# wg-perception/PartsBasedDetector

Measured on AMD Instinct MI355X. Metric: detect() frames/sec, 640x480, 26-part person model, higher is better.
Workload: dtype f32

## Files before the change

### partsbaseddetector_amd/csrc/k_conv_split32.hpp

```cpp
typedef __bf16 bf16x8 __attribute__((ext_vector_type(8)));
typedef _Float16 f16x8 __attribute__((ext_vector_type(8)));
typedef unsigned u32x4 __attribute__((ext_vector_type(4)));
typedef float f32x4 __attribute__((ext_vector_type(4)));
typedef float f32x16 __attribute__((ext_vector_type(16)));

template <int NT, int NW, int PIN, int NS = 3, bool MIX = false>
__global__ __launch_bounds__(64 * NW) __attribute__((amdgpu_waves_per_eu(1, PIN ? 1 : 2))) void k_conv_split32(const ConvTile* __restrict__ tiles, const LevelDev* __restrict__ levels,
                                                             const uint16_t* __restrict__ feat, const uint16_t* __restrict__ filt,
                                                             float* __restrict__ resp, int nf, int ntl_bank, int ntile0, int ngroups,
                                                             int ntiles_total, int kh, int kw, const float* __restrict__ oscale) {
  extern __shared__ __attribute__((aligned(16))) char smem[];
  using opnd = std::conditional_t<NS == 3, bf16x8, f16x8>;
  constexpr int ROWS = 4 * NW, NHALVES = 16 / ROWS, NTHR = 64 * NW, PPC = 4 * NS;
  const int TW = 16 + kw - 1, TH = ROWS + kh - 1, NC = TW * TH, PLANE = NC * 64;
  const int R = NHALVES * ngroups;
  const int lin = blockIdx.x;
  const int grp = lin / (8 * R), rem = lin - grp * (8 * R);
  const int tile_i = grp * 8 + (rem & 7), role = rem >> 3;
  if (tile_i >= ntiles_total) return;
  const int half = role & (NHALVES - 1), ngroup = role / NHALVES;
  const ConvTile t = tiles[tile_i];
  const LevelDev lv = levels[t.level];
  const int H = lv.ch, W = lv.cw;
  const int ty0 = t.y0 + ROWS * half, tx0 = t.x0;
  if (ty0 >= H) return;
  const int tid = threadIdx.x, lane = tid & 63, wave = __builtin_amdgcn_readfirstlane(tid >> 6);
  const uint16_t* F = feat + lv.cell_off * (NS * PBD_FLEN);
  {
    const int NPC = NC * PPC, oy = ty0 - kh / 2, ox = tx0 - kw / 2;
    constexpr unsigned ONE = NS == 3 ? 0x3F800000u : 0x6C000000u;
    auto cell_of = [](int i) { return NS == 3 ? (int)(((unsigned)i * 43691u) >> 19) : i >> 3; };
    const unsigned magic_tw = 0xFFFFFFFFu / (unsigned)TW + 1u;
    constexpr int BATCH = 12;
    for (int i0 = 0; i0 < NPC; i0 += NTHR * BATCH) {
      u32x4 v[BATCH];
#pragma unroll
      for (int j = 0; j < BATCH; ++j) {
        const int i = min(i0 + j * NTHR + tid, NPC - 1);
        const int cell = cell_of(i), piece = i - cell * PPC;
        const int cy = (int)__umulhi((unsigned)cell, magic_tw), cx = cell - cy * TW;
        const int y = min(max(oy + cy, 0), H - 1), x = min(max(ox + cx, 0), W - 1);
        v[j] = *(const u32x4*)(F + ((size_t)(y * W + x) * (NS * PBD_FLEN) + piece * 8));
      }
#pragma unroll
      for (int j = 0; j < BATCH; ++j) {
        const int i = i0 + j * NTHR + tid;
        if (i < NPC) {
          const int cell = cell_of(i), piece = i - cell * PPC;
          const int cy = (int)__umulhi((unsigned)cell, magic_tw), cx = cell - cy * TW;
          const int y = oy + cy, x = ox + cx;
          const bool inside = y >= 0 && y < H && x >= 0 && x < W;
          const u32x4 border = u32x4{0u, 0u, 0u, piece == 3 ? ONE : 0u};
          const int q = piece & 3;
          *(u32x4*)(smem + (piece >> 2) * PLANE + cell * 64 + ((q ^ ((cell >> 2) & 3)) << 4)) = inside ? v[j] : border;
        }
      }
    }
  }
  __syncthreads();
  const int c = lane & 31, kg = lane >> 5;
  const int mid = ((c & 15) >= 4 && (c & 15) < 12) ? 1 : 0;
  const int pos = (c & 15) + 16 * (mid ^ (c >> 4));
  const int vw = min(16, W - tx0), vh = min(ROWS, H - ty0), ncell = vw * vh;
  const int nmt = (ncell + 31) >> 5;
  const int mvalid = __builtin_amdgcn_readfirstlane(max(0, min(2, (nmt - wave + NW - 1) / NW)));
  const unsigned vw_magic = 65535u / (unsigned)vw + 1u;
  int cl0[2], cofs[2];
  bool cval[2];
#pragma unroll
  for (int m = 0; m < 2; ++m) {
    const int idx = 32 * (wave + NW * m) + pos;
    cval[m] = idx < ncell;
    const int ic = min(idx, ncell - 1);
    const int cy = (int)(((unsigned)ic * vw_magic) >> 16), cx = ic - cy * vw;
    cl0[m] = cy * TW + cx;
    cofs[m] = (ty0 + cy) * W + tx0 + cx;
  }
  const int ntb = ntile0 + ngroup * NT;
  f32x16 acc[NT][2];
#pragma unroll
  for (int nt = 0; nt < NT; ++nt)
#pragma unroll
    for (int m = 0; m < 2; ++m)
#pragma unroll
      for (int r = 0; r < 16; ++r) acc[nt][m][r] = 0.f;
  const uint16_t* bl = filt + (size_t)ntb * 512 + lane * 8;
  const size_t bs_split = (size_t)ntl_bank * 512, bs_kstep = NS * bs_split;
  const int nkstep = 2 * kh * kw;
#ifdef PBD_BANK_PRIO
  __builtin_amdgcn_s_setprio(PBD_BANK_PRIO);
#endif

  auto k_loop = [&](auto mv_tag) __attribute__((always_inline)) {
    constexpr int MV = decltype(mv_tag)::value;
    auto load_b = [&](opnd (&b)[NT][NS], int kstep) __attribute__((always_inline)) {
      const uint16_t* p = bl + (size_t)min(kstep, nkstep - 1) * bs_kstep;
#pragma unroll
      for (int s = 0; s < NS; ++s)
#pragma unroll
        for (int nt = 0; nt < NT; ++nt) b[nt][s] = *(const opnd*)(p + s * bs_split + nt * 512);
    };
    auto load_a = [&](opnd (&a)[2][NS], int tapofs, int ks) __attribute__((always_inline)) {
#pragma unroll
      for (int m = 0; m < MV; ++m) {
        const int cl = cl0[m] + tapofs;
        const char* p = smem + cl * 64 + (((2 * ks + kg) ^ ((cl >> 2) & 3)) << 4);
#pragma unroll
        for (int s = 0; s < NS; ++s) a[m][s] = *(const opnd*)(p + s * PLANE);
      }
    };
    auto mma = [&](const opnd (&a)[2][NS], const opnd (&b)[NT][NS]) __attribute__((always_inline)) {
      auto sweep = [&](int sa, int sb) __attribute__((always_inline)) {
#pragma unroll
        for (int nt = 0; nt < NT; ++nt)
#pragma unroll
          for (int m = 0; m < MV; ++m) {
            if constexpr (NS == 3) acc[nt][m] = __builtin_amdgcn_mfma_f32_32x32x16_bf16(b[nt][sb], a[m][sa], acc[nt][m], 0, 0, 0);
            else acc[nt][m] = __builtin_amdgcn_mfma_f32_32x32x16_f16(b[nt][sb], a[m][sa], acc[nt][m], 0, 0, 0);
          }
      };
      if constexpr (NS == 3) { sweep(1, 1); sweep(0, 2); sweep(2, 0); }
      sweep(0, 1); sweep(1, 0); sweep(0, 0);
    };
    int ti = 0, tj = 0;
    const int ntap = kh * kw;
    opnd a0[2][NS], a1[2][NS], b0[NT][NS], b1[NT][NS];
    load_b(b0, 0);
    load_a(a0, 0, 0);
#pragma unroll 1
    for (int tap = 0; tap < ntap; ++tap) {
      const int tapofs = ti * TW + tj;
      auto deal = [&]() {
        if constexpr (PIN == 2) {
#pragma unroll
          for (int i = 0; i < NS * NT; ++i) { __builtin_amdgcn_sched_group_barrier(0x8, NS == 3 ? (MV == 2 ? 3 : 1) : MV, 0); __builtin_amdgcn_sched_group_barrier(0x20, 1, 0); }
#pragma unroll
          for (int i = 0; i < NS * MV; ++i) { __builtin_amdgcn_sched_group_barrier(0x8, 2, 0); __builtin_amdgcn_sched_group_barrier(0x100, 1, 0); }
        }
      };
      if (PIN) __builtin_amdgcn_sched_barrier(0);
      load_b(b1, 2 * tap + 1);
      load_a(a1, tapofs, 1);
      if (PIN == 1) __builtin_amdgcn_sched_barrier(0);
      mma(a0, b0);
      deal();
      if (PIN) __builtin_amdgcn_sched_barrier(0);
      if (++tj == kw) { tj = 0; ++ti; }
      const int nextofs = tap + 1 < ntap ? ti * TW + tj : tapofs;
      load_b(b0, 2 * tap + 2);
      load_a(a0, nextofs, 0);
      if (PIN == 1) __builtin_amdgcn_sched_barrier(0);
      mma(a1, b1);
      deal();
      if (PIN) __builtin_amdgcn_sched_barrier(0);
    }
  };
  if (mvalid == 2) k_loop(std::integral_constant<int, 2>());
  else if (mvalid == 1) k_loop(std::integral_constant<int, 1>());
  if (mvalid == 0) return;

  float* Rl = resp + lv.cell_off * nf;
  const size_t HW = (size_t)H * W;
  int nfw = nf;
  if constexpr (MIX) { Rl += (size_t)(t.pad & 0xFFFF) * HW; nfw = t.pad >> 16; }
#pragma unroll
  for (int m = 0; m < 2; ++m) {
    if (m < mvalid && cval[m]) {
#pragma unroll
      for (int nt = 0; nt < NT; ++nt) {
        float* pl = Rl + (size_t)(32 * (ntb + nt) + 4 * kg) * HW + cofs[m];
#pragma unroll
        for (int r = 0; r < 16; ++r) {
          const int fo = (r & 3) + 8 * (r >> 2);
          if (32 * (ntb + nt) + 4 * kg + fo < nfw) pl[(size_t)fo * HW] = NS == 3 ? acc[nt][m][r] : acc[nt][m][r] * oscale[32 * (ntb + nt) + 4 * kg + fo];
        }
      }
    }
  }
}

template <int NT, int NW, int PIN, int NS = 3, bool MIX = false>
static void launch_conv_split_t(const ConvTile* tiles, int ntiles, const LevelDev* levels, const uint16_t* feat_split, const uint16_t* wS,
                                float* resp, int nf, int ntl_bank, int ntile0, int ngroups, int kh, int kw, hipStream_t s, const float* oscale = nullptr,
                                int nf_stride = 0) {
  constexpr int ROWS = 4 * NW, NHALVES = 16 / ROWS;
  const size_t lds = (size_t)(16 + kw - 1) * (ROWS + kh - 1) * 64 * NS;
  static LdsOptIn optin;
  optin.ensure((const void*)k_conv_split32<NT, NW, PIN, NS, MIX>, lds);
  const int grid = (ntiles + 7) / 8 * 8 * NHALVES * ngroups;
  hipLaunchKernelGGL((k_conv_split32<NT, NW, PIN, NS, MIX>), dim3(grid), dim3(64 * NW), lds, s, tiles, levels, feat_split, wS, resp, MIX ? nf_stride : nf,
                     ntl_bank, ntile0, ngroups, ntiles, kh, kw, oscale);
}
template <int NW, int PIN, int NS, bool MIX = false>
static void launch_conv_split_groups(const ConvTile* tiles, int ntiles, const LevelDev* levels, const uint16_t* feat_split, const uint16_t* wS,
                                     float* resp, int nf, int kh, int kw, const float* oscale, hipStream_t s, int nf_stride = 0, int G = 5) {
  const int ntl = conv_split_ntiles(nf), full = ntl / G, rest = ntl - G * full;
  auto go = [&](int nt, int ntile0, int ngroups) {
    switch (nt) {
      case 1: launch_conv_split_t<1, NW, PIN, NS, MIX>(tiles, ntiles, levels, feat_split, wS, resp, nf, ntl, ntile0, ngroups, kh, kw, s, oscale, nf_stride); break;
      case 2: launch_conv_split_t<2, NW, PIN, NS, MIX>(tiles, ntiles, levels, feat_split, wS, resp, nf, ntl, ntile0, ngroups, kh, kw, s, oscale, nf_stride); break;
      case 3: launch_conv_split_t<3, NW, PIN, NS, MIX>(tiles, ntiles, levels, feat_split, wS, resp, nf, ntl, ntile0, ngroups, kh, kw, s, oscale, nf_stride); break;
      case 4: launch_conv_split_t<4, NW, PIN, NS, MIX>(tiles, ntiles, levels, feat_split, wS, resp, nf, ntl, ntile0, ngroups, kh, kw, s, oscale, nf_stride); break;
      case 5: launch_conv_split_t<5, NW, PIN, NS, MIX>(tiles, ntiles, levels, feat_split, wS, resp, nf, ntl, ntile0, ngroups, kh, kw, s, oscale, nf_stride); break;
      default: break;
    }
  };
  if (full) go(G, 0, full);
  if (rest) go(rest, G * full, 1);
}
```

### partsbaseddetector_amd/csrc/k_conv_split_variants.hip

```cpp
#include <algorithm>
#include <type_traits>
#include "pbd_internal.hpp"

int conv_split_ntiles(int nf);

namespace conv_variants {
#include "k_conv_split32.hpp"

template <int NT>
__device__ __forceinline__ void conv_split32p_body(char* smem, const ConvTile* __restrict__ tiles, const LevelDev* __restrict__ levels,
                                                   const uint16_t* __restrict__ feat, const uint16_t* __restrict__ filt,
                                                   float* __restrict__ resp, int nf, int ntl_bank, int ntile0, int ngroups,
                                                   int ntiles_total) {
  constexpr int NW = 4, KW = 5, TW = 20, NC = 400, HPLANE = NC * 32, HBUF = 3 * HPLANE, NTAP = 25, NHP = NC * 6;
  const int tid = threadIdx.x, lane = tid & 63, wave = __builtin_amdgcn_readfirstlane(tid >> 6);
  const int xcd = blockIdx.x & 7, j0 = blockIdx.x >> 3, nwx = gridDim.x >> 3;
  const int ntx = ntiles_total > xcd ? (ntiles_total - xcd + 7) >> 3 : 0;
  const int nunits = ntx * ngroups;
  if (j0 >= nunits) return;
  const int c = lane & 31, kg = lane >> 5;
  const int mid = ((c & 15) >= 4 && (c & 15) < 12) ? 1 : 0;
  const int pos = (c & 15) + 16 * (mid ^ (c >> 4));
  const size_t bs_split = (size_t)ntl_bank * 512, bs_kstep = 3 * bs_split;

  struct Unit { int y0, x0, W, H, ng; size_t cell_off; };
  auto unit_of = [&](int v) {
    const int ti = xcd + 8 * (v / ngroups);
    const ConvTile t = tiles[ti];
    const LevelDev lv = levels[t.level];
    return Unit{t.y0, t.x0, lv.cw, lv.ch, v - (v / ngroups) * ngroups, (size_t)lv.cell_off};
  };
  auto piece_src = [&](const Unit& U, int half, int jj) {
    const int i = min(jj * 256 + tid, NHP - 1);
    const int cell = (int)(((unsigned)i * 43691u) >> 18), p6 = i - cell * 6;
    const int cy = (int)(((unsigned)cell * 52429u) >> 20), cx = cell - cy * TW;
    const int y = min(max(U.y0 - 2 + cy, 0), U.H - 1), x = min(max(U.x0 - 2 + cx, 0), U.W - 1);
    const int gp = (p6 >> 1) * 4 + 2 * half + (p6 & 1);
    return (const u32x4*)(feat + (U.cell_off + (size_t)(y * U.W + x)) * (3 * PBD_FLEN) + gp * 8);
  };
  auto piece_put = [&](const Unit& U, int half, int jj, char* buf, u32x4 v) {
    const int i = min(jj * 256 + tid, NHP - 1);
    const int cell = (int)(((unsigned)i * 43691u) >> 18), p6 = i - cell * 6;
    const int cy = (int)(((unsigned)cell * 52429u) >> 20), cx = cell - cy * TW;
    const int y = U.y0 - 2 + cy, x = U.x0 - 2 + cx;
    const unsigned m = 0u - (unsigned)((int)(y >= 0) & (int)(y < U.H) & (int)(x >= 0) & (int)(x < U.W));
    const unsigned b3 = (half == 1 && p6 == 1) ? 0x3F800000u : 0u;
    const u32x4 w = u32x4{v[0] & m, v[1] & m, v[2] & m, (v[3] & m) | (b3 & ~m)};
    *(u32x4*)(buf + (p6 >> 1) * HPLANE + cell * 32 + (((p6 & 1) ^ ((cell >> 3) & 1)) << 4)) = w;
  };
  constexpr int NPT = (NHP + 255) / 256;
  static_assert(2 * NPT <= NTAP - 1, "a half tile is staged under the 25 k-steps of the previous half");

  int v = j0;
  Unit U = unit_of(v);
  {
    u32x4 r[NPT];
#pragma unroll
    for (int jj = 0; jj < NPT; ++jj) r[jj] = *piece_src(U, 0, jj);
#pragma unroll
    for (int jj = 0; jj < NPT; ++jj) piece_put(U, 0, jj, smem, r[jj]);
  }
  const uint16_t* bl = filt + (size_t)(ntile0 + U.ng * NT) * 512 + lane * 8;
  bf16x8 a0[2][3], a1[2][3], b0[NT][3], b1[NT][3];
  auto load_b = [&](bf16x8 (&b)[NT][3], const uint16_t* p) {
#pragma unroll
    for (int s = 0; s < 3; ++s)
#pragma unroll
      for (int nt = 0; nt < NT; ++nt) b[nt][s] = *(const bf16x8*)(p + s * bs_split + nt * 512);
  };
  load_b(b0, bl);
  f32x16 acc[NT][2];

  while (true) {
    const int vn = v + nwx;
    const bool has_next = vn < nunits;
    const Unit Un = unit_of(has_next ? vn : v);
    const uint16_t* bln = filt + (size_t)(ntile0 + Un.ng * NT) * 512 + lane * 8;
    const int vw = min(16, U.W - U.x0), vh = min(16, U.H - U.y0), ncell = vw * vh;
    const int nmt = (ncell + 31) >> 5;
    const int mvalid = __builtin_amdgcn_readfirstlane(max(0, min(2, (nmt - wave + NW - 1) / NW)));
    const unsigned vw_magic = 65535u / (unsigned)vw + 1u;
    int cl0[2], cofs[2];
    bool cval[2];
#pragma unroll
    for (int m = 0; m < 2; ++m) {
      const int idx = 32 * (wave + NW * m) + pos;
      cval[m] = idx < ncell;
      const int ic = min(idx, ncell - 1);
      const int cy = (int)(((unsigned)ic * vw_magic) >> 16), cx = ic - cy * vw;
      cl0[m] = cy * TW + cx;
      cofs[m] = (U.y0 + cy) * U.W + U.x0 + cx;
    }
#pragma unroll
    for (int nt = 0; nt < NT; ++nt)
#pragma unroll
      for (int m = 0; m < 2; ++m)
#pragma unroll
        for (int r = 0; r < 16; ++r) acc[nt][m][r] = 0.f;

    auto run_half = [&](auto mv_tag, int half, const char* bufc, char* bufn, const Unit& Us, int hs, const uint16_t* bnext,
                        bf16x8 (&ac)[2][3], bf16x8 (&bc)[NT][3], bf16x8 (&an)[2][3], bf16x8 (&bn)[NT][3]) __attribute__((always_inline)) {
      constexpr int MV = decltype(mv_tag)::value;
      auto load_a = [&](bf16x8 (&a)[2][3], int tapofs) {
#pragma unroll
        for (int m = 0; m < (MV ? MV : 1); ++m) {
          if (MV == 0) break;
          const int cl = cl0[m] + tapofs;
          const char* p = bufc + cl * 32 + ((kg ^ ((cl >> 3) & 1)) << 4);
#pragma unroll
          for (int s = 0; s < 3; ++s) a[m][s] = *(const bf16x8*)(p + s * HPLANE);
        }
      };
      auto mma = [&](const bf16x8 (&a)[2][3], const bf16x8 (&b)[NT][3]) {
        auto sweep = [&](int sa, int sb) {
#pragma unroll
          for (int nt = 0; nt < NT; ++nt)
#pragma unroll
            for (int m = 0; m < MV; ++m) acc[nt][m] = __builtin_amdgcn_mfma_f32_32x32x16_bf16(b[nt][sb], a[m][sa], acc[nt][m], 0, 0, 0);
        };
        sweep(1, 1); sweep(0, 2); sweep(2, 0); sweep(0, 1); sweep(1, 0); sweep(0, 0);
      };
      auto deal = [&](int extra_vmem, int extra_dsw) {
        if constexpr (MV > 0) {
#pragma unroll
          for (int i = 0; i < 3 * NT; ++i) { __builtin_amdgcn_sched_group_barrier(0x8, MV == 2 ? 3 : 1, 0); __builtin_amdgcn_sched_group_barrier(0x20, 1, 0); }
          if (extra_vmem) { __builtin_amdgcn_sched_group_barrier(0x8, 1, 0); __builtin_amdgcn_sched_group_barrier(0x20, 1, 0); }
          if (extra_dsw) { __builtin_amdgcn_sched_group_barrier(0x8, 1, 0); __builtin_amdgcn_sched_group_barrier(0x200, 1, 0); }
#pragma unroll
          for (int i = 0; i < 3 * MV; ++i) { __builtin_amdgcn_sched_group_barrier(0x8, MV == 2 ? 2 : 1, 0); __builtin_amdgcn_sched_group_barrier(0x100, 1, 0); }
        }
      };
      const uint16_t* bh = bl + (size_t)half * bs_kstep;
      __syncthreads();
      load_a(ac, 0);
      u32x4 pv = u32x4{0u, 0u, 0u, 0u};
      int ti = 0, tj = 0;
#pragma unroll 1
      for (int tp = 0; tp < NTAP / 2; ++tp) {
        __builtin_amdgcn_sched_barrier(0);
        pv = *piece_src(Us, hs, min(tp, NPT - 1));
        if (MV) load_b(bn, bh + (size_t)(2 * (2 * tp + 1)) * bs_kstep);
        if (++tj == KW) { tj = 0; ++ti; }
        load_a(an, ti * TW + tj);
        mma(ac, bc);
        deal(1, 0);
        __builtin_amdgcn_sched_barrier(0);
        piece_put(Us, hs, min(tp, NPT - 1), bufn, pv);
        if (MV) load_b(bc, bh + (size_t)(2 * (2 * tp + 2)) * bs_kstep);
        if (++tj == KW) { tj = 0; ++ti; }
        load_a(ac, ti * TW + tj);
        mma(an, bn);
        deal(0, 1);
        __builtin_amdgcn_sched_barrier(0);
      }
      __builtin_amdgcn_sched_barrier(0);
      if (MV) load_b(bn, bnext);
      mma(ac, bc);
      deal(0, 0);
      __builtin_amdgcn_sched_barrier(0);
    };
    auto run_unit = [&](auto mv_tag) __attribute__((always_inline)) {
      run_half(mv_tag, 0, smem, smem + HBUF, U, 1, bl + bs_kstep, a0, b0, a1, b1);
      run_half(mv_tag, 1, smem + HBUF, smem, Un, 0, bln, a1, b1, a0, b0);
    };
    run_unit(std::integral_constant<int, 2>());

    {
      float* Rl = resp + U.cell_off * nf;
      const size_t HW = (size_t)U.H * U.W;
      const int ntb = ntile0 + U.ng * NT;
#pragma unroll
      for (int m = 0; m < 2; ++m) {
        if (m < mvalid && cval[m]) {
#pragma unroll
          for (int nt = 0; nt < NT; ++nt) {
            float* pl = Rl + (size_t)(32 * (ntb + nt) + 4 * kg) * HW + cofs[m];
#pragma unroll
            for (int r = 0; r < 16; ++r) {
              const int fo = (r & 3) + 8 * (r >> 2);
              if (32 * (ntb + nt) + 4 * kg + fo < nf) pl[(size_t)fo * HW] = acc[nt][m][r];
            }
          }
        }
      }
    }
    if (!has_next) break;
    v = vn; U = Un; bl = bln;
  }
}

template <int NT>
__global__ __launch_bounds__(256) __attribute__((amdgpu_waves_per_eu(1, 1))) void k_conv_split32p(const ConvTile* __restrict__ tiles, const LevelDev* __restrict__ levels,
    const uint16_t* __restrict__ feat, const uint16_t* __restrict__ filt, float* __restrict__ resp, int nf, int ntl_bank, int ntile0, int ngroups, int ntiles_total) {
  extern __shared__ __attribute__((aligned(16))) char smem[];
  conv_split32p_body<NT>(smem, tiles, levels, feat, filt, resp, nf, ntl_bank, ntile0, ngroups, ntiles_total);
}
template <int NT>
static void launch_conv_split_p(const ConvTile* tiles, int ntiles, const LevelDev* levels, const uint16_t* feat_split, const uint16_t* wS,
                                float* resp, int nf, int ntl_bank, int ntile0, int ngroups, int ncu, hipStream_t s) {
  const size_t lds = 2 * 3 * 400 * 32;
  static LdsOptIn optin;
  optin.ensure((const void*)k_conv_split32p<NT>, lds);
  const int grid = 8 * std::max(1, (ncu + 7) / 8);
  hipLaunchKernelGGL((k_conv_split32p<NT>), dim3(grid), dim3(256), lds, s, tiles, levels, feat_split, wS, resp, nf, ntl_bank, ntile0, ngroups, ntiles);
}
static void launch_conv_split_persistent(const ConvTile* tiles, int ntiles, const LevelDev* levels, const uint16_t* feat_split, const uint16_t* wS,
                                         float* resp, int nf, int ncu, hipStream_t s) {
  const int ntl = conv_split_ntiles(nf), full = ntl / 5, rest = ntl - 5 * full;
  if (full) launch_conv_split_p<5>(tiles, ntiles, levels, feat_split, wS, resp, nf, ntl, 0, full, ncu, s);
  switch (rest) {
    case 1: launch_conv_split_p<1>(tiles, ntiles, levels, feat_split, wS, resp, nf, ntl, 5 * full, 1, ncu, s); break;
    case 2: launch_conv_split_p<2>(tiles, ntiles, levels, feat_split, wS, resp, nf, ntl, 5 * full, 1, ncu, s); break;
    case 3: launch_conv_split_p<3>(tiles, ntiles, levels, feat_split, wS, resp, nf, ntl, 5 * full, 1, ncu, s); break;
    case 4: launch_conv_split_p<4>(tiles, ntiles, levels, feat_split, wS, resp, nf, ntl, 5 * full, 1, ncu, s); break;
    default: break;
  }
}

}

void launch_conv_split_variant(const pbd_handle* h, int variant) {
  using namespace conv_variants;
  const pbd_model_desc& m = h->md;
  const ConvTile* tiles = h->d_conv_tiles;
  const LevelDev* levels = h->d_levels;
  const int ntiles = h->n_conv_tiles, nf = m.nfilters, kh = m.kh, kw = m.kw;
  const uint16_t* fs = h->d_feat_split, *wS = h->d_wS;
  const float* osc = h->d_split_oscale;
  float* resp = (float*)h->d_resp;
  hipStream_t s = h->stream;
  if (ntiles <= 0) return;
  if (h->conv_mode == PBD_CONV_SPLIT_F16) {
    if (variant == 4) launch_conv_split_groups<4, 0, 2>(tiles, ntiles, levels, fs, wS, resp, nf, kh, kw, osc, s);
    else launch_conv_split_groups<4, 2, 2>(tiles, ntiles, levels, fs, wS, resp, nf, kh, kw, osc, s, 0, variant == 7 ? 4 : variant == 8 ? 3 : 5);
  } else if (variant == 6 && kh == 5 && kw == 5) launch_conv_split_persistent(tiles, ntiles, levels, fs, wS, resp, nf, h->ncu, s);
  else if (variant == 1) launch_conv_split_groups<4, 1, 3>(tiles, ntiles, levels, fs, wS, resp, nf, kh, kw, nullptr, s);
  else if (variant == 2) launch_conv_split_groups<2, 2, 3>(tiles, ntiles, levels, fs, wS, resp, nf, kh, kw, nullptr, s);
  else if (variant == 3) launch_conv_split_groups<2, 1, 3>(tiles, ntiles, levels, fs, wS, resp, nf, kh, kw, nullptr, s);
  else if (variant == 4) launch_conv_split_groups<4, 0, 3>(tiles, ntiles, levels, fs, wS, resp, nf, kh, kw, nullptr, s);
  else if (variant == 5) launch_conv_split_groups<2, 0, 3>(tiles, ntiles, levels, fs, wS, resp, nf, kh, kw, nullptr, s);
  else launch_conv_split_groups<4, 2, 3>(tiles, ntiles, levels, fs, wS, resp, nf, kh, kw, nullptr, s, 0, variant == 7 ? 4 : variant == 8 ? 3 : 5);
}
```

Before: 2447.

## Switch split-precision conv kernel from 32x32 to 16x16 MFMA with interleaved filter prefetch

Rewrites the main split-bf16 convolution inner loop to use 16x16x32 MFMA instructions in inline asm, with four 16-cell M tiles per wave instead of two 32-cell tiles. Filter loads for the next tap are spread between MFMA groups under explicit scheduling barriers, and activations for the next tap are loaded from LDS after the last filter tile. The epilogue now writes 4 outputs per accumulator, and accumulator hazards are padded with s_nop. The variants file keeps the old 32x32 kernel under a new header so other variants are unaffected. The aim is finer M granularity on partial tiles and better overlap of global loads with matrix work, at the cost of more MFMA instructions and hand-written scheduling.

```diff
diff --git a/partsbaseddetector_amd/csrc/k_conv_split32.hpp b/partsbaseddetector_amd/csrc/k_conv_split32.hpp
--- a/partsbaseddetector_amd/csrc/k_conv_split32.hpp
+++ b/partsbaseddetector_amd/csrc/k_conv_split32.hpp
@@ -10,7 +10,6 @@
                                                              float* __restrict__ resp, int nf, int ntl_bank, int ntile0, int ngroups,
                                                              int ntiles_total, int kh, int kw, const float* __restrict__ oscale) {
   extern __shared__ __attribute__((aligned(16))) char smem[];
-  using opnd = std::conditional_t<NS == 3, bf16x8, f16x8>;
   constexpr int ROWS = 4 * NW, NHALVES = 16 / ROWS, NTHR = 64 * NW, PPC = 4 * NS;
   const int TW = 16 + kw - 1, TH = ROWS + kh - 1, NC = TW * TH, PLANE = NC * 64;
   const int R = NHALVES * ngroups;
@@ -58,18 +57,19 @@
     }
   }
   __syncthreads();
-  const int c = lane & 31, kg = lane >> 5;
-  const int mid = ((c & 15) >= 4 && (c & 15) < 12) ? 1 : 0;
-  const int pos = (c & 15) + 16 * (mid ^ (c >> 4));
+  const int col = lane & 15, kb = lane >> 4;
+  const bool inner = col >= 4 && col < 12;
+  const int kk = inner ? col - 4 : col < 4 ? col : col - 8;
+  const int pos = ((kk >> 1) << 2) + (inner ? 0 : 2) + (kk & 1);
   const int vw = min(16, W - tx0), vh = min(ROWS, H - ty0), ncell = vw * vh;
-  const int nmt = (ncell + 31) >> 5;
-  const int mvalid = __builtin_amdgcn_readfirstlane(max(0, min(2, (nmt - wave + NW - 1) / NW)));
+  const int nmt = (ncell + 15) >> 4;
+  const int mvalid = __builtin_amdgcn_readfirstlane(max(0, min(4, (nmt - wave + NW - 1) / NW)));
   const unsigned vw_magic = 65535u / (unsigned)vw + 1u;
-  int cl0[2], cofs[2];
-  bool cval[2];
-#pragma unroll
-  for (int m = 0; m < 2; ++m) {
-    const int idx = 32 * (wave + NW * m) + pos;
+  int cl0[4], cofs[4];
+  bool cval[4];
+#pragma unroll
+  for (int m = 0; m < 4; ++m) {
+    const int idx = 16 * (wave + NW * m) + pos;
     cval[m] = idx < ncell;
     const int ic = min(idx, ncell - 1);
     const int cy = (int)(((unsigned)ic * vw_magic) >> 16), cx = ic - cy * vw;
@@ -77,105 +77,128 @@
     cofs[m] = (ty0 + cy) * W + tx0 + cx;
   }
   const int ntb = ntile0 + ngroup * NT;
-  f32x16 acc[NT][2];
-#pragma unroll
-  for (int nt = 0; nt < NT; ++nt)
-#pragma unroll
-    for (int m = 0; m < 2; ++m)
-#pragma unroll
-      for (int r = 0; r < 16; ++r) acc[nt][m][r] = 0.f;
-  const uint16_t* bl = filt + (size_t)ntb * 512 + lane * 8;
-  const size_t bs_split = (size_t)ntl_bank * 512, bs_kstep = NS * bs_split;
-  const int nkstep = 2 * kh * kw;
+  const size_t bs_split = (size_t)ntl_bank * 512, bs_kstep = NS * bs_split, bs_tap = 2 * bs_kstep;
+  const uint16_t* bl = filt + (size_t)ntb * 512 + (size_t)(kb >> 1) * bs_kstep + (kb & 1) * 256 + col * 8;
 #ifdef PBD_BANK_PRIO
   __builtin_amdgcn_s_setprio(PBD_BANK_PRIO);
 #endif
 
+  constexpr int NTRI = NS == 3 ? 2 : 1;
+  auto mfma3 = [](int tri, f32x4& d, const u32x4 (&fb)[NS], const u32x4 (&fa)[NS]) __attribute__((always_inline)) {
+    if constexpr (NS == 3) {
+      if (tri == 0)
+        asm volatile("v_mfma_f32_16x16x32_bf16 %0, %1, %2, %0\n\tv_mfma_f32_16x16x32_bf16 %0, %3, %4, %0\n\tv_mfma_f32_16x16x32_bf16 %0, %5, %6, %0"
+                     : "+a"(d) : "v"(fb[1]), "v"(fa[1]), "v"(fb[2]), "v"(fa[0]), "v"(fb[0]), "v"(fa[2]));
+      else
+        asm volatile("v_mfma_f32_16x16x32_bf16 %0, %1, %2, %0\n\tv_mfma_f32_16x16x32_bf16 %0, %3, %4, %0\n\tv_mfma_f32_16x16x32_bf16 %0, %3, %2, %0"
+                     : "+a"(d) : "v"(fb[1]), "v"(fa[0]), "v"(fb[0]), "v"(fa[1]));
+    } else {
+      asm volatile("v_mfma_f32_16x16x32_f16 %0, %1, %2, %0\n\tv_mfma_f32_16x16x32_f16 %0, %3, %4, %0\n\tv_mfma_f32_16x16x32_f16 %0, %3, %2, %0"
+                   : "+a"(d) : "v"(fb[1]), "v"(fa[0]), "v"(fb[0]), "v"(fa[1]));
+    }
+  };
+
   auto k_loop = [&](auto mv_tag) __attribute__((always_inline)) {
-    constexpr int MV = decltype(mv_tag)::value;
-    auto load_b = [&](opnd (&b)[NT][NS], int kstep) __attribute__((always_inline)) {
-      const uint16_t* p = bl + (size_t)min(kstep, nkstep - 1) * bs_kstep;
-#pragma unroll
-      for (int s = 0; s < NS; ++s)
-#pragma unroll
-        for (int nt = 0; nt < NT; ++nt) b[nt][s] = *(const opnd*)(p + s * bs_split + nt * 512);
-    };
-    auto load_a = [&](opnd (&a)[2][NS], int tapofs, int ks) __attribute__((always_inline)) {
-#pragma unroll
-      for (int m = 0; m < MV; ++m) {
-        const int cl = cl0[m] + tapofs;
-        const char* p = smem + cl * 64 + (((2 * ks + kg) ^ ((cl >> 2) & 3)) << 4);
-#pragma unroll
-        for (int s = 0; s < NS; ++s) a[m][s] = *(const opnd*)(p + s * PLANE);
-      }
-    };
-    auto mma = [&](const opnd (&a)[2][NS], const opnd (&b)[NT][NS]) __attribute__((always_inline)) {
-      auto sweep = [&](int sa, int sb) __attribute__((always_inline)) {
-#pragma unroll
-        for (int nt = 0; nt < NT; ++nt)
+    constexpr int MV = decltype(mv_tag)::value, NU = 2 * MV * NTRI, NLD = 2 * NS, LPT = (NLD + NU - 2) / (NU - 1);
+    static_assert(NU >= 2 && LPT * (NU - 1) >= NLD, "a step's statements carry the next step's filter loads");
+    u32x4 a[4][NS], b[2][2][NS];
+    f32x4 acc[2 * NT][MV];
+#pragma unroll
+    for (int ft = 0; ft < 2 * NT; ++ft)
+#pragma unroll
+      for (int m = 0; m < MV; ++m) acc[ft][m] = f32x4{0.f, 0.f, 0.f, 0.f};
+    auto pad_acc = [&]() __attribute__((always_inline)) {
+#pragma unroll
+      for (int ft = 0; ft < 2 * NT; ++ft)
+#pragma unroll
+        for (int m = 0; m < MV; ++m) asm volatile("s_nop 7" : "+a"(acc[ft][m]));
+    };
+    auto ld_a = [&](int m, int tapofs) __attribute__((always_inline)) {
+      const int cl = cl0[m] + tapofs;
+      const char* p = smem + cl * 64 + ((kb ^ ((cl >> 2) & 3)) << 4);
+#pragma unroll
+      for (int s = 0; s < NS; ++s) a[m][s] = *(const u32x4*)(p + s * PLANE);
+    };
+    auto tap_body = [&](auto p_tag, const uint16_t* pt, const uint16_t* pn, int nextofs) __attribute__((always_inline)) {
+      constexpr int P = decltype(p_tag)::value;
+#pragma unroll
+      for (int nt = 0; nt < NT; ++nt) {
+        const int slot = (P + nt) & 1;
+        const bool last = nt == NT - 1;
+        const uint16_t* pl = last ? pn : pt + (nt + 1) * 512;
+#pragma unroll
+        for (int h = 0; h < 2; ++h)
 #pragma unroll
           for (int m = 0; m < MV; ++m) {
-            if constexpr (NS == 3) acc[nt][m] = __builtin_amdgcn_mfma_f32_32x32x16_bf16(b[nt][sb], a[m][sa], acc[nt][m], 0, 0, 0);
-            else acc[nt][m] = __builtin_amdgcn_mfma_f32_32x32x16_f16(b[nt][sb], a[m][sa], acc[nt][m], 0, 0, 0);
+#pragma unroll
+            for (int q = 0; q < NTRI; ++q) {
+              const int u = (h * MV + m) * NTRI + q;
+              mfma3(q + 2 - NTRI, acc[2 * nt + h][m], b[slot][h], a[m]);
+              if (u * LPT < NLD) {
+                __builtin_amdgcn_sched_barrier(0);
+#pragma unroll
+                for (int k = u * LPT; k < (u + 1) * LPT && k < NLD; ++k)
+                  b[slot ^ 1][k / NS][k % NS] = *(const u32x4*)(pl + (k % NS) * bs_split + (k / NS) * 128);
+                __builtin_amdgcn_sched_barrier(0);
+              }
+            }
+            if (last && h == 1) {
+              __builtin_amdgcn_sched_barrier(0);
+              ld_a(m, nextofs);
+              __builtin_amdgcn_sched_barrier(0);
+            }
           }
-      };
-      if constexpr (NS == 3) { sweep(1, 1); sweep(0, 2); sweep(2, 0); }
-      sweep(0, 1); sweep(1, 0); sweep(0, 0);
-    };
+      }
+    };
+    const int ntap = kh * kw;
+#pragma unroll
+    for (int k = 0; k < NLD; ++k) b[0][k / NS][k % NS] = *(const u32x4*)(bl + (k % NS) * bs_split + (k / NS) * 128);
+#pragma unroll
+    for (int m = 0; m < MV; ++m) ld_a(m, 0);
+    pad_acc();
     int ti = 0, tj = 0;
-    const int ntap = kh * kw;
-    opnd a0[2][NS], a1[2][NS], b0[NT][NS], b1[NT][NS];
-    load_b(b0, 0);
-    load_a(a0, 0, 0);
+    const uint16_t* pt = bl;
+    auto one_tap = [&](auto p_tag, int tap) __attribute__((always_inline)) {
+      if (++tj == kw) { tj = 0; ++ti; }
+      const bool more = tap + 1 < ntap;
+      const uint16_t* pn = more ? pt + bs_tap : pt;
+      tap_body(p_tag, pt, pn, more ? ti * TW + tj : 0);
+      pt = pn;
+    };
 #pragma unroll 1
-    for (int tap = 0; tap < ntap; ++tap) {
-      const int tapofs = ti * TW + tj;
-      auto deal = [&]() {
-        if constexpr (PIN == 2) {
-#pragma unroll
-          for (int i = 0; i < NS * NT; ++i) { __builtin_amdgcn_sched_group_barrier(0x8, NS == 3 ? (MV == 2 ? 3 : 1) : MV, 0); __builtin_amdgcn_sched_group_barrier(0x20, 1, 0); }
-#pragma unroll
-          for (int i = 0; i < NS * MV; ++i) { __builtin_amdgcn_sched_group_barrier(0x8, 2, 0); __builtin_amdgcn_sched_group_barrier(0x100, 1, 0); }
+    for (int tap = 0; tap < ntap; tap += 1 + (NT & 1)) {
+      one_tap(std::integral_constant<int, 0>(), tap);
+      if constexpr (NT & 1) {
+        if (tap + 1 >= ntap) break;
+        one_tap(std::integral_constant<int, 1>(), tap + 1);
+      }
+    }
+    pad_acc();
+
+    float* Rl = resp + lv.cell_off * nf;
+    const size_t HW = (size_t)H * W;
+    int nfw = nf;
+    if constexpr (MIX) { Rl += (size_t)(t.pad & 0xFFFF) * HW; nfw = t.pad >> 16; }
+#pragma unroll
+    for (int m = 0; m < MV; ++m) {
+      if (cval[m]) {
+#pragma unroll
+        for (int ft = 0; ft < 2 * NT; ++ft) {
+          const int f0 = 32 * ntb + 16 * ft + 4 * kb;
+          float* pl = Rl + (size_t)f0 * HW + cofs[m];
+#pragma unroll
+          for (int r = 0; r < 4; ++r)
+            if (f0 + r < nfw) pl[(size_t)r * HW] = NS == 3 ? acc[ft][m][r] : acc[ft][m][r] * oscale[f0 + r];
         }
-      };
-      if (PIN) __builtin_amdgcn_sched_barrier(0);
-      load_b(b1, 2 * tap + 1);
-      load_a(a1, tapofs, 1);
-      if (PIN == 1) __builtin_amdgcn_sched_barrier(0);
-      mma(a0, b0);
-      deal();
-      if (PIN) __builtin_amdgcn_sched_barrier(0);
-      if (++tj == kw) { tj = 0; ++ti; }
-      const int nextofs = tap + 1 < ntap ? ti * TW + tj : tapofs;
-      load_b(b0, 2 * tap + 2);
-      load_a(a0, nextofs, 0);
-      if (PIN == 1) __builtin_amdgcn_sched_barrier(0);
-      mma(a1, b1);
-      deal();
-      if (PIN) __builtin_amdgcn_sched_barrier(0);
+      }
     }
   };
-  if (mvalid == 2) k_loop(std::integral_constant<int, 2>());
-  else if (mvalid == 1) k_loop(std::integral_constant<int, 1>());
-  if (mvalid == 0) return;
-
-  float* Rl = resp + lv.cell_off * nf;
-  const size_t HW = (size_t)H * W;
-  int nfw = nf;
-  if constexpr (MIX) { Rl += (size_t)(t.pad & 0xFFFF) * HW; nfw = t.pad >> 16; }
-#pragma unroll
-  for (int m = 0; m < 2; ++m) {
-    if (m < mvalid && cval[m]) {
-#pragma unroll
-      for (int nt = 0; nt < NT; ++nt) {
-        float* pl = Rl + (size_t)(32 * (ntb + nt) + 4 * kg) * HW + cofs[m];
-#pragma unroll
-        for (int r = 0; r < 16; ++r) {
-          const int fo = (r & 3) + 8 * (r >> 2);
-          if (32 * (ntb + nt) + 4 * kg + fo < nfw) pl[(size_t)fo * HW] = NS == 3 ? acc[nt][m][r] : acc[nt][m][r] * oscale[32 * (ntb + nt) + 4 * kg + fo];
-        }
-      }
-    }
+  switch (mvalid) {
+    case 4: k_loop(std::integral_constant<int, 4>()); break;
+    case 3: k_loop(std::integral_constant<int, 3>()); break;
+    case 2: k_loop(std::integral_constant<int, 2>()); break;
+    case 1: k_loop(std::integral_constant<int, 1>()); break;
+    default: return;
   }
 }
 
diff --git a/partsbaseddetector_amd/csrc/k_conv_split32_m32.hpp b/partsbaseddetector_amd/csrc/k_conv_split32_m32.hpp
--- /dev/null
+++ b/partsbaseddetector_amd/csrc/k_conv_split32_m32.hpp
@@ -0,0 +1,210 @@
+typedef __bf16 bf16x8 __attribute__((ext_vector_type(8)));
+typedef _Float16 f16x8 __attribute__((ext_vector_type(8)));
+typedef unsigned u32x4 __attribute__((ext_vector_type(4)));
+typedef float f32x4 __attribute__((ext_vector_type(4)));
+typedef float f32x16 __attribute__((ext_vector_type(16)));
+
+template <int NT, int NW, int PIN, int NS = 3, bool MIX = false>
+__global__ __launch_bounds__(64 * NW) __attribute__((amdgpu_waves_per_eu(1, PIN ? 1 : 2))) void k_conv_split32(const ConvTile* __restrict__ tiles, const LevelDev* __restrict__ levels,
+                                                             const uint16_t* __restrict__ feat, const uint16_t* __restrict__ filt,
+                                                             float* __restrict__ resp, int nf, int ntl_bank, int ntile0, int ngroups,
+                                                             int ntiles_total, int kh, int kw, const float* __restrict__ oscale) {
+  extern __shared__ __attribute__((aligned(16))) char smem[];
+  using opnd = std::conditional_t<NS == 3, bf16x8, f16x8>;
+  constexpr int ROWS = 4 * NW, NHALVES = 16 / ROWS, NTHR = 64 * NW, PPC = 4 * NS;
+  const int TW = 16 + kw - 1, TH = ROWS + kh - 1, NC = TW * TH, PLANE = NC * 64;
+  const int R = NHALVES * ngroups;
+  const int lin = blockIdx.x;
+  const int grp = lin / (8 * R), rem = lin - grp * (8 * R);
+  const int tile_i = grp * 8 + (rem & 7), role = rem >> 3;
+  if (tile_i >= ntiles_total) return;
+  const int half = role & (NHALVES - 1), ngroup = role / NHALVES;
+  const ConvTile t = tiles[tile_i];
+  const LevelDev lv = levels[t.level];
+  const int H = lv.ch, W = lv.cw;
+  const int ty0 = t.y0 + ROWS * half, tx0 = t.x0;
+  if (ty0 >= H) return;
+  const int tid = threadIdx.x, lane = tid & 63, wave = __builtin_amdgcn_readfirstlane(tid >> 6);
+  const uint16_t* F = feat + lv.cell_off * (NS * PBD_FLEN);
+  {
+    const int NPC = NC * PPC, oy = ty0 - kh / 2, ox = tx0 - kw / 2;
+    constexpr unsigned ONE = NS == 3 ? 0x3F800000u : 0x6C000000u;
+    auto cell_of = [](int i) { return NS == 3 ? (int)(((unsigned)i * 43691u) >> 19) : i >> 3; };
+    const unsigned magic_tw = 0xFFFFFFFFu / (unsigned)TW + 1u;
+    constexpr int BATCH = 12;
+    for (int i0 = 0; i0 < NPC; i0 += NTHR * BATCH) {
+      u32x4 v[BATCH];
+#pragma unroll
+      for (int j = 0; j < BATCH; ++j) {
+        const int i = min(i0 + j * NTHR + tid, NPC - 1);
+        const int cell = cell_of(i), piece = i - cell * PPC;
+        const int cy = (int)__umulhi((unsigned)cell, magic_tw), cx = cell - cy * TW;
+        const int y = min(max(oy + cy, 0), H - 1), x = min(max(ox + cx, 0), W - 1);
+        v[j] = *(const u32x4*)(F + ((size_t)(y * W + x) * (NS * PBD_FLEN) + piece * 8));
+      }
+#pragma unroll
+      for (int j = 0; j < BATCH; ++j) {
+        const int i = i0 + j * NTHR + tid;
+        if (i < NPC) {
+          const int cell = cell_of(i), piece = i - cell * PPC;
+          const int cy = (int)__umulhi((unsigned)cell, magic_tw), cx = cell - cy * TW;
+          const int y = oy + cy, x = ox + cx;
+          const bool inside = y >= 0 && y < H && x >= 0 && x < W;
+          const u32x4 border = u32x4{0u, 0u, 0u, piece == 3 ? ONE : 0u};
+          const int q = piece & 3;
+          *(u32x4*)(smem + (piece >> 2) * PLANE + cell * 64 + ((q ^ ((cell >> 2) & 3)) << 4)) = inside ? v[j] : border;
+        }
+      }
+    }
+  }
+  __syncthreads();
+  const int c = lane & 31, kg = lane >> 5;
+  const int mid = ((c & 15) >= 4 && (c & 15) < 12) ? 1 : 0;
+  const int pos = (c & 15) + 16 * (mid ^ (c >> 4));
+  const int vw = min(16, W - tx0), vh = min(ROWS, H - ty0), ncell = vw * vh;
+  const int nmt = (ncell + 31) >> 5;
+  const int mvalid = __builtin_amdgcn_readfirstlane(max(0, min(2, (nmt - wave + NW - 1) / NW)));
+  const unsigned vw_magic = 65535u / (unsigned)vw + 1u;
+  int cl0[2], cofs[2];
+  bool cval[2];
+#pragma unroll
+  for (int m = 0; m < 2; ++m) {
+    const int idx = 32 * (wave + NW * m) + pos;
+    cval[m] = idx < ncell;
+    const int ic = min(idx, ncell - 1);
+    const int cy = (int)(((unsigned)ic * vw_magic) >> 16), cx = ic - cy * vw;
+    cl0[m] = cy * TW + cx;
+    cofs[m] = (ty0 + cy) * W + tx0 + cx;
+  }
+  const int ntb = ntile0 + ngroup * NT;
+  f32x16 acc[NT][2];
+#pragma unroll
+  for (int nt = 0; nt < NT; ++nt)
+#pragma unroll
+    for (int m = 0; m < 2; ++m)
+#pragma unroll
+      for (int r = 0; r < 16; ++r) acc[nt][m][r] = 0.f;
+  const uint16_t* bl = filt + (size_t)ntb * 512 + lane * 8;
+  const size_t bs_split = (size_t)ntl_bank * 512, bs_kstep = NS * bs_split;
+  const int nkstep = 2 * kh * kw;
+#ifdef PBD_BANK_PRIO
+  __builtin_amdgcn_s_setprio(PBD_BANK_PRIO);
+#endif
+
+  auto k_loop = [&](auto mv_tag) __attribute__((always_inline)) {
+    constexpr int MV = decltype(mv_tag)::value;
+    auto load_b = [&](opnd (&b)[NT][NS], int kstep) __attribute__((always_inline)) {
+      const uint16_t* p = bl + (size_t)min(kstep, nkstep - 1) * bs_kstep;
+#pragma unroll
+      for (int s = 0; s < NS; ++s)
+#pragma unroll
+        for (int nt = 0; nt < NT; ++nt) b[nt][s] = *(const opnd*)(p + s * bs_split + nt * 512);
+    };
+    auto load_a = [&](opnd (&a)[2][NS], int tapofs, int ks) __attribute__((always_inline)) {
+#pragma unroll
+      for (int m = 0; m < MV; ++m) {
+        const int cl = cl0[m] + tapofs;
+        const char* p = smem + cl * 64 + (((2 * ks + kg) ^ ((cl >> 2) & 3)) << 4);
+#pragma unroll
+        for (int s = 0; s < NS; ++s) a[m][s] = *(const opnd*)(p + s * PLANE);
+      }
+    };
+    auto mma = [&](const opnd (&a)[2][NS], const opnd (&b)[NT][NS]) __attribute__((always_inline)) {
+      auto sweep = [&](int sa, int sb) __attribute__((always_inline)) {
+#pragma unroll
+        for (int nt = 0; nt < NT; ++nt)
+#pragma unroll
+          for (int m = 0; m < MV; ++m) {
+            if constexpr (NS == 3) acc[nt][m] = __builtin_amdgcn_mfma_f32_32x32x16_bf16(b[nt][sb], a[m][sa], acc[nt][m], 0, 0, 0);
+            else acc[nt][m] = __builtin_amdgcn_mfma_f32_32x32x16_f16(b[nt][sb], a[m][sa], acc[nt][m], 0, 0, 0);
+          }
+      };
+      if constexpr (NS == 3) { sweep(1, 1); sweep(0, 2); sweep(2, 0); }
+      sweep(0, 1); sweep(1, 0); sweep(0, 0);
+    };
+    int ti = 0, tj = 0;
+    const int ntap = kh * kw;
+    opnd a0[2][NS], a1[2][NS], b0[NT][NS], b1[NT][NS];
+    load_b(b0, 0);
+    load_a(a0, 0, 0);
+#pragma unroll 1
+    for (int tap = 0; tap < ntap; ++tap) {
+      const int tapofs = ti * TW + tj;
+      auto deal = [&]() {
+        if constexpr (PIN == 2) {
+#pragma unroll
+          for (int i = 0; i < NS * NT; ++i) { __builtin_amdgcn_sched_group_barrier(0x8, NS == 3 ? (MV == 2 ? 3 : 1) : MV, 0); __builtin_amdgcn_sched_group_barrier(0x20, 1, 0); }
+#pragma unroll
+          for (int i = 0; i < NS * MV; ++i) { __builtin_amdgcn_sched_group_barrier(0x8, 2, 0); __builtin_amdgcn_sched_group_barrier(0x100, 1, 0); }
+        }
+      };
+      if (PIN) __builtin_amdgcn_sched_barrier(0);
+      load_b(b1, 2 * tap + 1);
+      load_a(a1, tapofs, 1);
+      if (PIN == 1) __builtin_amdgcn_sched_barrier(0);
+      mma(a0, b0);
+      deal();
+      if (PIN) __builtin_amdgcn_sched_barrier(0);
+      if (++tj == kw) { tj = 0; ++ti; }
+      const int nextofs = tap + 1 < ntap ? ti * TW + tj : tapofs;
+      load_b(b0, 2 * tap + 2);
+      load_a(a0, nextofs, 0);
+      if (PIN == 1) __builtin_amdgcn_sched_barrier(0);
+      mma(a1, b1);
+      deal();
+      if (PIN) __builtin_amdgcn_sched_barrier(0);
+    }
+  };
+  if (mvalid == 2) k_loop(std::integral_constant<int, 2>());
+  else if (mvalid == 1) k_loop(std::integral_constant<int, 1>());
+  if (mvalid == 0) return;
+
+  float* Rl = resp + lv.cell_off * nf;
+  const size_t HW = (size_t)H * W;
+  int nfw = nf;
+  if constexpr (MIX) { Rl += (size_t)(t.pad & 0xFFFF) * HW; nfw = t.pad >> 16; }
+#pragma unroll
+  for (int m = 0; m < 2; ++m) {
+    if (m < mvalid && cval[m]) {
+#pragma unroll
+      for (int nt = 0; nt < NT; ++nt) {
+        float* pl = Rl + (size_t)(32 * (ntb + nt) + 4 * kg) * HW + cofs[m];
+#pragma unroll
+        for (int r = 0; r < 16; ++r) {
+          const int fo = (r & 3) + 8 * (r >> 2);
+          if (32 * (ntb + nt) + 4 * kg + fo < nfw) pl[(size_t)fo * HW] = NS == 3 ? acc[nt][m][r] : acc[nt][m][r] * oscale[32 * (ntb + nt) + 4 * kg + fo];
+        }
+      }
+    }
+  }
+}
+
+template <int NT, int NW, int PIN, int NS = 3, bool MIX = false>
+static void launch_conv_split_t(const ConvTile* tiles, int ntiles, const LevelDev* levels, const uint16_t* feat_split, const uint16_t* wS,
+                                float* resp, int nf, int ntl_bank, int ntile0, int ngroups, int kh, int kw, hipStream_t s, const float* oscale = nullptr,
+                                int nf_stride = 0) {
+  constexpr int ROWS = 4 * NW, NHALVES = 16 / ROWS;
+  const size_t lds = (size_t)(16 + kw - 1) * (ROWS + kh - 1) * 64 * NS;
+  static LdsOptIn optin;
+  optin.ensure((const void*)k_conv_split32<NT, NW, PIN, NS, MIX>, lds);
+  const int grid = (ntiles + 7) / 8 * 8 * NHALVES * ngroups;
+  hipLaunchKernelGGL((k_conv_split32<NT, NW, PIN, NS, MIX>), dim3(grid), dim3(64 * NW), lds, s, tiles, levels, feat_split, wS, resp, MIX ? nf_stride : nf,
+                     ntl_bank, ntile0, ngroups, ntiles, kh, kw, oscale);
+}
+template <int NW, int PIN, int NS, bool MIX = false>
+static void launch_conv_split_groups(const ConvTile* tiles, int ntiles, const LevelDev* levels, const uint16_t* feat_split, const uint16_t* wS,
+                                     float* resp, int nf, int kh, int kw, const float* oscale, hipStream_t s, int nf_stride = 0, int G = 5) {
+  const int ntl = conv_split_ntiles(nf), full = ntl / G, rest = ntl - G * full;
+  auto go = [&](int nt, int ntile0, int ngroups) {
+    switch (nt) {
+      case 1: launch_conv_split_t<1, NW, PIN, NS, MIX>(tiles, ntiles, levels, feat_split, wS, resp, nf, ntl, ntile0, ngroups, kh, kw, s, oscale, nf_stride); break;
+      case 2: launch_conv_split_t<2, NW, PIN, NS, MIX>(tiles, ntiles, levels, feat_split, wS, resp, nf, ntl, ntile0, ngroups, kh, kw, s, oscale, nf_stride); break;
+      case 3: launch_conv_split_t<3, NW, PIN, NS, MIX>(tiles, ntiles, levels, feat_split, wS, resp, nf, ntl, ntile0, ngroups, kh, kw, s, oscale, nf_stride); break;
+      case 4: launch_conv_split_t<4, NW, PIN, NS, MIX>(tiles, ntiles, levels, feat_split, wS, resp, nf, ntl, ntile0, ngroups, kh, kw, s, oscale, nf_stride); break;
+      case 5: launch_conv_split_t<5, NW, PIN, NS, MIX>(tiles, ntiles, levels, feat_split, wS, resp, nf, ntl, ntile0, ngroups, kh, kw, s, oscale, nf_stride); break;
+      default: break;
+    }
+  };
+  if (full) go(G, 0, full);
+  if (rest) go(rest, G * full, 1);
+}
diff --git a/partsbaseddetector_amd/csrc/k_conv_split_variants.hip b/partsbaseddetector_amd/csrc/k_conv_split_variants.hip
--- a/partsbaseddetector_amd/csrc/k_conv_split_variants.hip
+++ b/partsbaseddetector_amd/csrc/k_conv_split_variants.hip
@@ -5,7 +5,7 @@
 int conv_split_ntiles(int nf);
 
 namespace conv_variants {
-#include "k_conv_split32.hpp"
+#include "k_conv_split32_m32.hpp"
 
 template <int NT>
 __device__ __forceinline__ void conv_split32p_body(char* smem, const ConvTile* __restrict__ tiles, const LevelDev* __restrict__ levels,
```

New measurement: 2590 (median of 6 runs). 1.06x the previous value.
